# Marcus-Forte/moptimizer_0

Measured on NVIDIA B200. Metric: point2point_linearized_residuals_per_sec, higher is better.
Workload: dtype f32

## Files before the change

moptimizer_0_b200/csrc/mopt_capi.cu:

```cuda
#include <dlfcn.h>

#include <cmath>
#include <atomic>
#include <chrono>
#include <cstdlib>
#include <cstring>
#include <mutex>

#include "mopt_internal.h"

using namespace mopt;

namespace {
thread_local std::string g_last_error;
}
namespace mopt {
void set_last_error(const std::string& msg) { g_last_error = msg; }
int store_upload_async(mopt_store* st, int group, const void* host, int host_dtype, int64_t host_stride, int64_t first,
                       int64_t count);
}

namespace {
struct NcclApi {
  typedef struct ncclComm* comm_t;
// ... 170 lines not shown

void fill_cost(const mopt_problem* p, CostDev* c) {
  std::memset(c, 0, sizeof(*c));
  c->model = p->model; c->variant = p->variant; c->P = p->num_parameters; c->O = p->num_outputs;
  c->jacobian = p->jacobian; c->loss = p->loss; c->has_cov = p->has_covariance ? 1 : 0;
  c->compute_dtype = p->compute_dtype; c->loss_param = p->loss_param;
  c->manifold = p->manifold;
  c->rot_offset = (p->model == MOPT_MODEL_POINT2POINT || p->model == MOPT_MODEL_PINHOLE ||
                   p->model == MOPT_MODEL_PINHOLE_DISTORT) ? 3 : -1;
  if (p->model >= MOPT_MODEL_USER_BASE) c->rot_offset = user_model_rot_offset(p->model);
  c->so3_guard = ((p->flags & MOPT_FLAG_REFERENCE_FLOAT_GUARD) && p->compute_dtype == MOPT_F32) ? kSo3GuardF32 : kSo3GuardF64;
  const int O = p->num_outputs;
  for (int i = 0; i < O * O; ++i) c->cov[i] = p->has_covariance ? p->covariance[i] : ((i % (O + 1) == 0) ? 1.0 : 0.0);
  std::memcpy(c->consts, p->consts, sizeof(c->consts));
}

int stage_cost(mopt_ctx* ctx, int i, const mopt_problem* p) {
  CostDev c;
  fill_cost(p, &c);
  if (ctx->cached_valid[i] && std::memcmp(&c, &ctx->cached_cost[i], sizeof(c)) == 0) return MOPT_OK;
  MOPT_CUDA_TRY(cudaStreamSynchronize(ctx->stream));
  ctx->h_slot->cost = c;
  MOPT_CUDA_TRY(cudaMemcpyAsync(&ctx->d_slots[i].cost, &ctx->h_slot->cost, sizeof(CostDev), cudaMemcpyHostToDevice, ctx->stream));
  MOPT_CUDA_TRY(cudaStreamSynchronize(ctx->stream));
  ctx->cached_cost[i] = c;
  ctx->cached_valid[i] = true;
  return MOPT_OK;
}

PassArgs make_args(mopt_ctx* ctx, const mopt_store* st, int slot, int accumulate, int mode_override) {
  PassArgs a;
  std::memset(&a, 0, sizeof(a));
  for (int s = 0; s < kMaxStreams; ++s) a.streams.p[s] = st->streams[s];
  a.n = st->n;
  a.pb = &ctx->d_slots[slot].pb;
  a.cost = &ctx->d_slots[slot].cost;
  a.partials = ctx->d_partials;
  a.ticket = ctx->d_ticket;
  a.out = ctx->d_trial;
  a.accumulate = accumulate;
  a.mode_ptr = &ctx->d_lm->pass_mode;
  a.mode_override = mode_override;
  a.masked = st->may_have_invalid ? 1 : 0;
  return a;
}

bool can_fuse_setup(const mopt_ctx* ctx, const mopt_problem* p, const mopt_store* st) {
  static const int env = [] {
    const char* e = getenv("MOPT_FUSED_SETUP");
    return (e && e[0]) ? (e[0] == '0' ? 0 : 1) : -1;
  }();
  if (env == 0) return false;
  if (p->model == MOPT_MODEL_EXP_CURVE && p->jacobian != MOPT_JAC_ANALYTICAL && st->dtype == MOPT_F32 &&
      p->compute_dtype == MOPT_F32 && !(p->flags & MOPT_FLAG_GENERIC_KERNEL) && !p->has_covariance &&
      !st->may_have_invalid && ctx->threads != 1024)
    return true;
  return p->model == MOPT_MODEL_POINT2POINT && p->jacobian == MOPT_JAC_ANALYTICAL &&
         p->manifold == MOPT_MANIFOLD_ADDITIVE;
}

int launch_pass(mopt_ctx* ctx, const mopt_store* st, const mopt_problem* p, int slot, int accumulate, int mode_override,
                bool push, const XArg* fused_x = nullptr) {
  PassArgs a = make_args(ctx, st, slot, accumulate, mode_override);
  if (fused_x) {
    a.fused_setup = 1;
    a.x = *fused_x;
  }
  if (push && ctx->world > 1 && ctx->peers_open && ctx->exchange_enabled) {
    for (int r = 0; r < ctx->world; ++r) a.peer.base[r] = ctx->peer_base[r];
    a.peer.world = ctx->world;
    a.peer.rank = ctx->rank;
    a.peer.push = 1;
    a.peer.fused = ctx->fused_consumer ? 1 : 0;
    a.peer.err = ctx->d_xerr;
    a.peer.err_dev = ctx->d_xerr_dev;
    a.peer.seq = ++ctx->xseq;
  }
  PassLaunch L{ctx->stream, ctx->num_sms, ctx->ctas_per_sm, ctx->threads};
  L.affine_fd = (p->compute_dtype == MOPT_F32) ? !(p->flags & MOPT_FLAG_GENERIC_KERNEL)
                                               : ((p->flags & MOPT_FLAG_STABLE_FD) && !(p->flags & MOPT_FLAG_GENERIC_KERNEL));
  L.identity_cov = !p->has_covariance;
  if (p->model >= MOPT_MODEL_USER_BASE)
    return launch_user(L, ctx->device, p->model, p->jacobian != MOPT_JAC_ANALYTICAL, st->dtype, p->compute_dtype, a);
  if (p->model == MOPT_MODEL_POINT2POINT && p->jacobian == MOPT_JAC_ANALYTICAL)
    return launch_p2p_moment(L, st->dtype, p->compute_dtype, p->loss,
                             p->variant == MOPT_P2P_EXACT || p->variant == MOPT_P2P_LEFT, a);
  if (p->model == MOPT_MODEL_POINT2POINT && !(p->flags & MOPT_FLAG_GENERIC_KERNEL) &&
      !(st->dtype == MOPT_F64 && p->compute_dtype == MOPT_F32))
    return launch_p2p_moment(L, st->dtype, p->compute_dtype, p->loss, false, a);
  if (p->model == MOPT_MODEL_PINHOLE_DISTORT) return launch_wide(L, p->model, st->dtype, p->compute_dtype, a);
  return launch_dense(L, p->model, p->jacobian != MOPT_JAC_ANALYTICAL, st->dtype, p->compute_dtype, a);
}

int allreduce_trial(mopt_ctx* ctx, int P, int mode_override) {
  if (ctx->world <= 1 || !ctx->exchange_enabled) return MOPT_OK;
  if (ctx->peers_open) {
    if (ctx->fused_consumer) return MOPT_OK;
    peer_reduce_kernel<<<1, 64, 0, ctx->stream>>>(ctx->d_xbuf, ctx->world, ctx->xseq, ctx->d_trial, packed_size(P),
                                                  &ctx->d_lm->pass_mode, mode_override, ctx->d_xerr, ctx->d_xerr_dev);
    MOPT_CUDA_TRY(cudaGetLastError());
    return MOPT_OK;
  }
  if (!ctx->nccl_comm) {
    set_last_error("sharded context has neither a NCCL communicator nor an open peer exchange");
    return MOPT_ERR_COMM;
  }
  MOPT_NCCL_TRY(nccl().AllReduce(ctx->d_trial, ctx->d_trial, size_t(packed_size(P)), kNcclFloat64, kNcclSum,
                                 static_cast<NcclApi::comm_t>(ctx->nccl_comm), ctx->stream));
  return MOPT_OK;
}

void unpack_result(const PassResult& r, int P, double* H, double* b, double* sum) {
  if (H)
    for (int i = 0; i < P; ++i)
// ... 10 lines not shown
int check_exchange_alive(const mopt_ctx* ctx) {
  if (ctx->h_xerr && *reinterpret_cast<volatile int*>(ctx->h_xerr)) {
    set_last_error("an earlier peer exchange on this context timed out (a rank died); destroy the context");
    return MOPT_ERR_COMM;
  }
  return MOPT_OK;
}

int enqueue_pass(mopt_ctx* ctx, mopt_store* st, const mopt_problem* p, const double* x, int mode) {
  MOPT_TRY(check_exchange_alive(ctx));
  MOPT_CUDA_TRY(cudaSetDevice(ctx->device));
  MOPT_TRY(stage_cost(ctx, 0, p));
  const int P = p->num_parameters;
  XArg xa;
  std::memset(&xa, 0, sizeof(xa));
  if (P > 0) {
    MOPT_REQUIRE(x != nullptr, "null parameter vector");
    for (int i = 0; i < P; ++i) xa.v[i] = x[i];
  }
  if (can_fuse_setup(ctx, p, st)) {
    MOPT_TRY(launch_pass(ctx, st, p, 0, 0, mode, true, &xa));
  } else {
    setup_kernel<<<1, 32, 0, ctx->stream>>>(&ctx->d_slots[0], xa);
    MOPT_CUDA_TRY(cudaGetLastError());
    if (user_model_has_setup(p->model))
      MOPT_TRY(launch_user_setup(ctx->stream, ctx->device, p->model, &ctx->d_slots[0], nullptr, xa.v, P));
    MOPT_TRY(launch_pass(ctx, st, p, 0, 0, mode, true));
  }
  MOPT_TRY(allreduce_trial(ctx, P, mode));
  return MOPT_OK;
}

}

namespace mopt {
int setup_slot(mopt_ctx* ctx, int slot, const mopt_problem* problem, const double* x) {
  MOPT_TRY(stage_cost(ctx, slot, problem));
  XArg xa;
  std::memset(&xa, 0, sizeof(xa));
  for (int i = 0; i < problem->num_parameters; ++i) xa.v[i] = x[i];
  setup_kernel<<<1, 32, 0, ctx->stream>>>(&ctx->d_slots[slot], xa);
  MOPT_CUDA_TRY(cudaGetLastError());
  if (user_model_has_setup(problem->model))
    MOPT_TRY(launch_user_setup(ctx->stream, ctx->device, problem->model, &ctx->d_slots[slot], nullptr, xa.v,
                               problem->num_parameters));
  return MOPT_OK;
}
}

namespace {

int fetch_result(mopt_ctx* ctx, int P, double* H, double* b, double* sum) {
  MOPT_CUDA_TRY(cudaMemcpyAsync(ctx->h_result, ctx->d_trial, sizeof(double) * packed_size(P), cudaMemcpyDeviceToHost, ctx->stream));
  MOPT_CUDA_TRY(cudaStreamSynchronize(ctx->stream));
  if (ctx->h_xerr && *reinterpret_cast<volatile int*>(ctx->h_xerr)) {
    set_last_error("peer exchange timed out waiting for another rank");
    return MOPT_ERR_COMM;
  }
  unpack_result(*ctx->h_result, P, H, b, sum);
  return MOPT_OK;
}

int finish_lm(mopt_ctx* ctx, int P, double* x, mopt_lm_report* report, bool on_host = false) {
  LmState* hs = ctx->h_lm;
  constexpr int kFirstTrials = 48;
  const size_t first = offsetof(LmState, trials) + sizeof(mopt_lm_trial) * kFirstTrials;
  if (!on_host) {
    MOPT_CUDA_TRY(cudaMemcpyAsync(hs, ctx->d_lm, first, cudaMemcpyDeviceToHost, ctx->stream));
    MOPT_CUDA_TRY(cudaStreamSynchronize(ctx->stream));
  }
  if (!on_host && hs->num_trials > kFirstTrials) {
    const int more = (hs->num_trials < MOPT_MAX_TRACE ? hs->num_trials : MOPT_MAX_TRACE) - kFirstTrials;
    MOPT_CUDA_TRY(cudaMemcpyAsync(reinterpret_cast<char*>(hs) + first, reinterpret_cast<const char*>(ctx->d_lm) + first,
                                  sizeof(mopt_lm_trial) * size_t(more), cudaMemcpyDeviceToHost, ctx->stream));
    MOPT_CUDA_TRY(cudaStreamSynchronize(ctx->stream));
  }
// ... 286 lines not shown

int mopt_lm_minimize(mopt_ctx* ctx, int n_costs, mopt_store* const* stores, const mopt_problem* problems,
                     const mopt_lm_options* options, double* x, mopt_lm_report* report) try {
  MOPT_REQUIRE(ctx && stores && problems && x && report, "null argument");
  if (n_costs <= 0) {
    set_last_error("No cost function added!");
    return MOPT_ERR_INVALID_ARGUMENT;
  }
  MOPT_REQUIRE(n_costs <= MOPT_MAX_COSTS, "too many cost terms");
  mopt_lm_options opt;
  if (options) opt = *options; else mopt_lm_default_options(&opt);
  MOPT_REQUIRE(opt.max_iterations >= 0, "Optimization::max_iterations cannot be less than 0.");
  MOPT_REQUIRE(opt.lm_max_iterations >= 0, "lm_max_iterations cannot be negative");
  const int P = problems[0].num_parameters;
  MOPT_REQUIRE(P > 0 && P <= kMaxP, "bad num_parameters");
  for (int c = 0; c < n_costs; ++c) {
    MOPT_REQUIRE(stores[c] && stores[c]->ctx == ctx, "store does not belong to this context");
    MOPT_TRY(validate_problem(stores[c], &problems[c], true));
    MOPT_REQUIRE(problems[c].num_parameters == P, "all cost terms must share the parameter vector");
    MOPT_REQUIRE(problems[c].manifold == problems[0].manifold, "all cost terms must use the same manifold");
  }
  MOPT_TRY(check_exchange_alive(ctx));
  MOPT_CUDA_TRY(cudaSetDevice(ctx->device));
  std::memset(report, 0, offsetof(mopt_lm_report, trials));
  if (opt.max_iterations == 0) {
    report->status = MOPT_MAXIMUM_ITERATIONS_REACHED;
    return MOPT_OK;
  }
  for (int c = 0; c < n_costs; ++c) MOPT_TRY(stage_cost(ctx, c, &problems[c]));

  LmInit in;
  std::memset(&in, 0, sizeof(in));
  in.P = P; in.n_costs = n_costs; in.max_it = opt.max_iterations; in.lm_max_it = opt.lm_max_iterations;
  in.speculative = opt.speculative ? 1 : 0; in.scalar_f32 = (opt.scalar_dtype == MOPT_F32) ? 1 : 0;
  bool has_update = false;
  for (int c = 0; c < n_costs; ++c) has_update = has_update || (stores[c]->index != nullptr);
  if (has_update) in.speculative = 0;
  in.lambda_factor = opt.lambda_factor;
  in.flags = opt.flags;
  for (int i = 0; i < P; ++i) in.x0[i] = x[i];
  bool init_launched = false;
  auto launch_init = [&]() -> int {
    if (init_launched) return MOPT_OK;
    lm_init_kernel<<<1, 32, 0, ctx->stream>>>(ctx->d_lm, ctx->d_slots, in);
    MOPT_CUDA_TRY(cudaGetLastError());
    init_launched = true;
// ... 214 lines not shown
```

moptimizer_0_b200/csrc/mopt_icp.cu:

```cuda
#include <cmath>
#include <cstring>
#include <vector>

#include "mopt_internal.h"

using namespace mopt;

struct mopt_nn_index {
  mopt_ctx* ctx = nullptr;
  int dtype = MOPT_F64;
  int64_t m = 0;
  double max_dist = 0.0, cell = 0.0;
  double origin[3] = {0, 0, 0};
  int dims[3] = {1, 1, 1};
  int64_t ncells = 1;
  void* d_pts = nullptr;
  int* d_orig = nullptr;
  unsigned int* d_start = nullptr;
  long long* d_matched = nullptr;
};

namespace {

struct GridDesc {
// ... 154 lines not shown
    if (best_pos != 0xffffffffu) {
      tx[i] = ST(px[best_pos]);
      ty[i] = ST(py[best_pos]);
      tz[i] = ST(pz[best_pos]);
      ++local;
    } else {
      const ST no_match = ST(__longlong_as_double(0x7ff8000000000000LL));
      tx[i] = no_match;
      ty[i] = no_match;
      tz[i] = no_match;
    }
  }
  for (int off = 16; off >= 1; off >>= 1) local += __shfl_xor_sync(0xffffffffu, local, off);
  if ((threadIdx.x & 31) == 0 && local) atomicAdd(reinterpret_cast<unsigned long long*>(matched), (unsigned long long)local);
}

template <typename T>
int build_index(mopt_nn_index* ix, const void* host, int host_dtype) {
  mopt_ctx* ctx = ix->ctx;
  const int64_t m = ix->m;
  const size_t esz = sizeof(T);
  T* d_aos = nullptr;
  MOPT_CUDA_TRY(cudaMalloc(&d_aos, esz * 3 * size_t(m > 0 ? m : 1)));
  if ((host_dtype == MOPT_F32) == (sizeof(T) == 4)) {
    MOPT_CUDA_TRY(cudaMemcpyAsync(d_aos, host, esz * 3 * size_t(m), cudaMemcpyHostToDevice, ctx->stream));
  } else {
    std::vector<T> tmp(size_t(m) * 3);
    if (host_dtype == MOPT_F32) { const float* h = static_cast<const float*>(host); for (size_t i = 0; i < tmp.size(); ++i) tmp[i] = T(h[i]); }
    else { const double* h = static_cast<const double*>(host); for (size_t i = 0; i < tmp.size(); ++i) tmp[i] = T(h[i]); }
    MOPT_CUDA_TRY(cudaMemcpyAsync(d_aos, tmp.data(), esz * 3 * size_t(m), cudaMemcpyHostToDevice, ctx->stream));
    MOPT_CUDA_TRY(cudaStreamSynchronize(ctx->stream));
  }
  const int bb_blocks = 296;
  double* d_part = nullptr;
  MOPT_CUDA_TRY(cudaMalloc(&d_part, sizeof(double) * 6 * bb_blocks));
  bbox_kernel<T><<<bb_blocks, 256, 0, ctx->stream>>>(d_aos, m, d_part);
  MOPT_CUDA_TRY(cudaGetLastError());
  std::vector<double> part(6 * bb_blocks);
  MOPT_CUDA_TRY(cudaMemcpyAsync(part.data(), d_part, sizeof(double) * part.size(), cudaMemcpyDeviceToHost, ctx->stream));
  MOPT_CUDA_TRY(cudaStreamSynchronize(ctx->stream));
  cudaFree(d_part);
  double lo[3] = {1e300, 1e300, 1e300}, hi[3] = {-1e300, -1e300, -1e300};
  for (int b = 0; b < bb_blocks; ++b)
    for (int k = 0; k < 3; ++k) {
      lo[k] = std::fmin(lo[k], part[b * 6 + k]);
      hi[k] = std::fmax(hi[k], part[b * 6 + 3 + k]);
// ... 50 lines not shown

template <typename ST, typename T>
void launch_reassoc(mopt_store* st, mopt_nn_index* ix, const ParamBlock* pb, const LmState* gate) {
  GridDesc g;
  for (int k = 0; k < 3; ++k) { g.origin[k] = ix->origin[k]; g.dims[k] = ix->dims[k]; }
  g.inv_cell = 1.0 / ix->cell;
  const T* pts = static_cast<const T*>(ix->d_pts);
  int blocks = int(std::min<int64_t>((st->n + 255) / 256, 148 * 32));
  if (blocks < 1) blocks = 1;
  reassociate_kernel<ST, T><<<blocks, 256, 0, st->ctx->stream>>>(
      static_cast<const ST*>(st->streams[0]), static_cast<const ST*>(st->streams[1]), static_cast<const ST*>(st->streams[2]),
      static_cast<ST*>(st->streams[3]), static_cast<ST*>(st->streams[4]), static_cast<ST*>(st->streams[5]), st->n, pb, g,
      ix->max_dist, pts, pts + ix->m, pts + 2 * ix->m, ix->d_orig, ix->d_start, ix->d_matched, gate);
}

}

namespace mopt {

int enqueue_reassociate(mopt_store* st, const ParamBlock* pb, const LmState* gate) {
  mopt_nn_index* ix = st->index;
  if (!ix) return MOPT_OK;
  MOPT_CUDA_TRY(cudaMemsetAsync(ix->d_matched, 0, sizeof(long long), st->ctx->stream));
  if (st->dtype == MOPT_F32 && ix->dtype == MOPT_F32) launch_reassoc<float, float>(st, ix, pb, gate);
  else if (st->dtype == MOPT_F32 && ix->dtype == MOPT_F64) launch_reassoc<float, double>(st, ix, pb, gate);
  else if (st->dtype == MOPT_F64 && ix->dtype == MOPT_F32) launch_reassoc<double, float>(st, ix, pb, gate);
  else launch_reassoc<double, double>(st, ix, pb, gate);
  MOPT_CUDA_TRY(cudaGetLastError());
  st->may_have_invalid = true;
  return MOPT_OK;
}

}

extern "C" {

int mopt_nn_index_create(mopt_ctx* ctx, const void* host_xyz, int host_dtype, int index_dtype, int64_t m,
                         double max_distance, mopt_nn_index** out) try {
  MOPT_REQUIRE(ctx && out && (host_xyz || m == 0), "null argument");
  MOPT_REQUIRE(m >= 0 && m < (int64_t(1) << 31), "target cloud size must be below 2^31");
  MOPT_REQUIRE(max_distance > 0.0 && std::isfinite(max_distance), "max_distance must be positive");
  MOPT_REQUIRE((host_dtype == MOPT_F32 || host_dtype == MOPT_F64) && (index_dtype == MOPT_F32 || index_dtype == MOPT_F64),
               "bad dtype");
  MOPT_CUDA_TRY(cudaSetDevice(ctx->device));
  mopt_nn_index* ix = new mopt_nn_index();
  ix->ctx = ctx;
// ... 53 lines not shown
```

moptimizer_0_b200/csrc/mopt_internal.h:

```cpp
#pragma once

#include <cuda_runtime.h>

#include "mopt_common.cuh"
#include "mopt_lm.cuh"
#include "mopt_lm_mono.cuh"
#include "mopt_models.cuh"
#include "mopt_pass.cuh"

struct mopt_ctx {
  int device = 0;
  int num_sms = 148;
  cudaStream_t stream = nullptr;
  cudaStream_t copy_stream = nullptr;
  double* d_partials = nullptr;
  unsigned int* d_ticket = nullptr;
  mopt::PassResult* d_trial = nullptr;
  mopt::CostSlot* d_slots = nullptr;
  mopt::LmState* d_lm = nullptr;
  mopt::PassResult* h_result = nullptr;
  mopt::LmState* h_lm = nullptr;
  mopt::LmState* d_lm_host = nullptr;
  mopt::CostSlot* h_slot = nullptr;
  int* h_flags = nullptr;
// ... 1 lines not shown
  int flags_capacity = 0;
  mopt::CostDev cached_cost[MOPT_MAX_COSTS];
  bool cached_valid[MOPT_MAX_COSTS] = {false};
  void* d_stage[2] = {nullptr, nullptr};
  size_t stage_bytes = 0;
  cudaEvent_t ev_copy[2] = {nullptr, nullptr};
  cudaEvent_t ev_free[2] = {nullptr, nullptr};
  cudaEvent_t ev_batch[2] = {nullptr, nullptr};
  int ctas_per_sm = 0;
  int threads = 0;
  void* nccl_comm = nullptr;
  int rank = 0, world = 1;
  mopt::XSlot* d_xbuf = nullptr;
  mopt::XSlot* peer_base[mopt::kMaxWorld] = {nullptr};
  bool peers_open = false;
  bool exchange_enabled = true;
  bool fused_consumer = true;
  unsigned long long xseq = 0;
  int* h_xerr = nullptr;
  int* d_xerr = nullptr;
  unsigned long long* d_gen = nullptr;
  unsigned long long mono_gen = 0;
  int* d_xerr_dev = nullptr;
};

struct mopt_store {
  mopt_ctx* ctx = nullptr;
  int model = 0;
  int dtype = 0;
  int64_t n = 0;
  int nstreams = 0;
  void* streams[mopt::kMaxStreams] = {nullptr};
  struct mopt_nn_index* index = nullptr;
  bool may_have_invalid = false;
};

namespace mopt {

struct PassLaunch {
  cudaStream_t stream;
  int num_sms;
  int ctas_per_sm;
  int threads;
  bool affine_fd = true;
  bool identity_cov = false;
};

int launch_p2p_moment(const PassLaunch& L, int store_dtype, int compute_dtype, int loss, bool qrot, const PassArgs& a);
int launch_p2p_moment_gen2(const PassLaunch& L, int loss, bool qrot, const PassArgs& a);
int launch_p2p_lm_mono(const PassLaunch& L, int store_dtype, int compute_dtype, int loss, bool qrot, const PassArgs& a,
                       const MonoArgs& m);
int launch_dense(const PassLaunch& L, int model, bool numeric, int store_dtype, int compute_dtype, const PassArgs& a);

int setup_slot(mopt_ctx* ctx, int slot, const mopt_problem* problem, const double* x);
int enqueue_reassociate(mopt_store* st, const ParamBlock* pb, const LmState* gate);

int launch_wide(const PassLaunch& L, int model, int store_dtype, int compute_dtype, const PassArgs& a);

int launch_user(const PassLaunch& L, int device, int model, bool numeric, int store_dtype, int compute_dtype,
                const PassArgs& a);
int launch_user_setup(cudaStream_t stream, int device, int model, CostSlot* slot, const double* x_dev,
                      const double* x_host, int P);
int user_model_rot_offset(int model);
bool user_model_has_setup(int model);

int pick_grid(const void* kernel, int threads, const PassLaunch& L, int64_t work_items);

}
```

moptimizer_0_b200/csrc/mopt_pass_p2p2.cu:

```cuda
#include "mopt_internal.h"
#include "mopt_pass_p2p2.cuh"

namespace mopt {
namespace {

struct ShapeGen2 {
  static constexpr int THREADS = 384, STAGES = 2, U = 2, FLUSH = 16;
};

template <int LOSS, bool QROT, bool MASKED, bool FUSED, class S>
int launch_gen2_one(const PassLaunch& L, const PassArgs& a0) {
  auto kern = p2p_moment2_kernel<LOSS, QROT, MASKED, FUSED, S::THREADS, 1, S::STAGES, S::U, S::FLUSH, 0>;
  constexpr size_t smem = p2p2_ring_bytes(S::THREADS, S::STAGES, S::U);
  static bool configured[64] = {false};
  int dev = 0;
  MOPT_CUDA_TRY(cudaGetDevice(&dev));
  if (dev < 0 || dev >= 64 || !configured[dev]) {
    MOPT_CUDA_TRY(cudaFuncSetAttribute(kern, cudaFuncAttributeMaxDynamicSharedMemorySize, int(smem)));
    if (dev >= 0 && dev < 64) configured[dev] = true;
  }
  PassArgs a = a0;
  for (int k = 0; k < 6; ++k)
    if (reinterpret_cast<uintptr_t>(a.streams.p[k]) & 15u) a.no_ring = 1;
  const int64_t groups = a.n / 4;
  int64_t grid = int64_t(L.ctas_per_sm > 0 ? L.ctas_per_sm : 1) * L.num_sms;
  if (grid > L.num_sms) grid = L.num_sms;
  const int64_t need = (groups + S::THREADS - 1) / S::THREADS;
  if (need < grid) grid = need;
  if (grid < 1) grid = 1;
  kern<<<int(grid), S::THREADS, smem, L.stream>>>(a);
  MOPT_CUDA_TRY(cudaGetLastError());
  return MOPT_OK;
}

template <int LOSS, bool QROT, class S>
int launch_gen2_flags(const PassLaunch& L, const PassArgs& a) {
  if (a.masked)
    return a.fused_setup ? launch_gen2_one<LOSS, QROT, true, true, S>(L, a) : launch_gen2_one<LOSS, QROT, true, false, S>(L, a);
  return a.fused_setup ? launch_gen2_one<LOSS, QROT, false, true, S>(L, a) : launch_gen2_one<LOSS, QROT, false, false, S>(L, a);
}

template <class S>
int launch_gen2(const PassLaunch& L, int loss, bool qrot, const PassArgs& a) {
  switch (loss) {
    case MOPT_LOSS_NONE:
      return qrot ? launch_gen2_flags<MOPT_LOSS_NONE, true, S>(L, a) : launch_gen2_flags<MOPT_LOSS_NONE, false, S>(L, a);
    case MOPT_LOSS_GEMAN_MCCLURE:
      return qrot ? launch_gen2_flags<MOPT_LOSS_GEMAN_MCCLURE, true, S>(L, a)
                  : launch_gen2_flags<MOPT_LOSS_GEMAN_MCCLURE, false, S>(L, a);
    case MOPT_LOSS_HUBER:
      return qrot ? launch_gen2_flags<MOPT_LOSS_HUBER, true, S>(L, a) : launch_gen2_flags<MOPT_LOSS_HUBER, false, S>(L, a);
    default:
      set_last_error("unknown loss kind");
      return MOPT_ERR_INVALID_ARGUMENT;
// ... 11 lines not shown
```

moptimizer_0_b200/csrc/mopt_pass_p2p2.cuh:

```cuda
#pragma once

#include "mopt_pass.cuh"

namespace mopt {
#ifdef __CUDACC__

__device__ __forceinline__ float2 bc2(float a) { return make_float2(a, a); }
__device__ __forceinline__ float2 neg2(float2 a) { return make_float2(-a.x, -a.y); }
__device__ __forceinline__ float2 fma2(float2 a, float2 b, float2 c) { return __ffma2_rn(a, b, c); }
__device__ __forceinline__ float2 add2(float2 a, float2 b) { return __fadd2_rn(a, b); }
__device__ __forceinline__ float2 sub2(float2 a, float2 b) { return __fadd2_rn(a, neg2(b)); }
__device__ __forceinline__ float2 mul2(float2 a, float2 b) { return __fmul2_rn(a, b); }

__device__ __forceinline__ unsigned smem_u32(const void* p) { return static_cast<unsigned>(__cvta_generic_to_shared(p)); }
__device__ __forceinline__ void mbar_init(uint64_t* bar, unsigned count) {
  asm volatile("mbarrier.init.shared::cta.b64 [%0], %1;" ::"r"(smem_u32(bar)), "r"(count) : "memory");
}
__device__ __forceinline__ void mbar_expect_tx(uint64_t* bar, unsigned bytes) {
  asm volatile("mbarrier.arrive.expect_tx.shared::cta.b64 _, [%0], %1;" ::"r"(smem_u32(bar)), "r"(bytes) : "memory");
}
__device__ __forceinline__ void mbar_arrive(uint64_t* bar) {
  asm volatile("mbarrier.arrive.shared::cta.b64 _, [%0];" ::"r"(smem_u32(bar)) : "memory");
}
__device__ __forceinline__ void mbar_wait(uint64_t* bar, unsigned parity) {
  asm volatile(
      "{\n"
      ".reg .pred p;\n"
      "MOPT_WAIT:\n"
      "mbarrier.try_wait.parity.shared::cta.b64 p, [%0], %1;\n"
      "@p bra MOPT_DONE;\n"
      "bra MOPT_WAIT;\n"
      "MOPT_DONE:\n"
      "}\n" ::"r"(smem_u32(bar)),
      "r"(parity)
      : "memory");
}
__device__ __forceinline__ void bulk_g2s(void* dst, const void* src, unsigned bytes, uint64_t* bar) {
  asm volatile("cp.async.bulk.shared::cluster.global.mbarrier::complete_tx::bytes [%0], [%1], %2, [%3];" ::"r"(smem_u32(dst)),
               "l"(src), "r"(bytes), "r"(smem_u32(bar))
               : "memory");
}

template <int LOSS>
__device__ __forceinline__ float loss_weight_fast(float k, float e2) {
  if constexpr (LOSS == MOPT_LOSS_HUBER) {
    float rs;
    asm("rsqrt.approx.ftz.f32 %0, %1;" : "=f"(rs) : "f"(fmaxf(e2, 1.17549435e-38f)));
    return (e2 <= k * k) ? 1.0f : k * rs;
  } else {
    return loss_weight<float>(LOSS, k, e2);
  }
}

template <int LOSS, bool QROT, bool MASKED>
__device__ __forceinline__ void p2p_moments_x2(const float (&R)[9], const float (&t)[3], float lossp, float2 px, float2 py,
                                               float2 pz, float2 yx, float2 yy, float2 yz, float2 (&acc)[kP2PRaw]) {
  bool skip0 = false, skip1 = false;
  if constexpr (MASKED) {
    skip0 = yx.x != yx.x; skip1 = yx.y != yx.y;
    if (skip0) { px.x = py.x = pz.x = 0.f; yx.x = t[0]; yy.x = t[1]; yz.x = t[2]; }
    if (skip1) { px.y = py.y = pz.y = 0.f; yx.y = t[0]; yy.y = t[1]; yz.y = t[2]; }
  }
  const float2 q0 = fma2(px, bc2(R[0]), fma2(py, bc2(R[1]), mul2(pz, bc2(R[2]))));
  const float2 q1 = fma2(px, bc2(R[3]), fma2(py, bc2(R[4]), mul2(pz, bc2(R[5]))));
// ... 21 lines not shown
  acc[19] = fma2(w2, r0, acc[19]); acc[20] = fma2(w2, r1, acc[20]); acc[21] = fma2(w2, r2, acc[21]);
  acc[22] = add2(acc[22], e2);
}

template <bool MASKED>
__device__ __forceinline__ void p2p_cost_x2(const float (&R)[9], const float (&t)[3], float2 px, float2 py, float2 pz,
                                            float2 yx, float2 yy, float2 yz, float2 (&acc)[kP2PRaw]) {
  const float2 r0 = sub2(add2(fma2(px, bc2(R[0]), fma2(py, bc2(R[1]), mul2(pz, bc2(R[2])))), bc2(t[0])), yx);
  const float2 r1 = sub2(add2(fma2(px, bc2(R[3]), fma2(py, bc2(R[4]), mul2(pz, bc2(R[5])))), bc2(t[1])), yy);
  const float2 r2 = sub2(add2(fma2(px, bc2(R[6]), fma2(py, bc2(R[7]), mul2(pz, bc2(R[8])))), bc2(t[2])), yz);
  float2 e2 = fma2(r0, r0, fma2(r1, r1, mul2(r2, r2)));
  if constexpr (MASKED) {
    if (yx.x != yx.x) e2.x = 0.f;
    if (yx.y != yx.y) e2.y = 0.f;
  }
  acc[22] = add2(acc[22], e2);
}

constexpr size_t p2p2_ring_bytes(int threads, int stages, int u) { return size_t(stages) * 6 * size_t(u) * threads * 16; }

template <int LOSS, bool QROT, bool MASKED, bool FUSED, int THREADS, int MINB, int STAGES, int U, int FLUSH_ROUNDS,
          int PF = 0>
__global__ void __launch_bounds__(THREADS, MINB) p2p_moment2_kernel(const PassArgs a) {
  const int mode = a.mode_override >= 0 ? a.mode_override : *a.mode_ptr;
  if (mode == PASS_SKIP) return;
  if (peer_failed(a)) return;
  constexpr int NW = THREADS / 32;
  constexpr int CHUNK = THREADS * U;

  __shared__ double s_warp[NW * 32];
  __shared__ double s_tot[32];
  __shared__ double s_set0[FUSED ? 12 : 1];
  __shared__ __align__(8) uint64_t s_full[STAGES > 0 ? STAGES : 1];
  __shared__ __align__(8) uint64_t s_empty[STAGES > 0 ? STAGES : 1];
  extern __shared__ __align__(128) unsigned char p2p2_ring[];
  float4* ring = reinterpret_cast<float4*>(p2p2_ring);

  const int lane = threadIdx.x & 31;
  const double* set0 = FUSED ? s_set0 : a.pb->sets[0];
  if constexpr (FUSED) {
    if (threadIdx.x == 0) {
      double xl[6];
#pragma unroll
      for (int i = 0; i < 6; ++i) xl[i] = a.x.v[i];
      p2p_fused_set0(a.cost, xl, s_set0);
    }
// ... 135 lines not shown
    for (int64_t g = full_rounds * stride + int64_t(blockIdx.x) * THREADS + threadIdx.x; g < ngroups;
         g += int64_t(gridDim.x) * THREADS) {
      direct_group(g);
      if (++since_flush >= FLUSH_ROUNDS) {
        flush();
        since_flush = 0;
      }
    }
    if (blockIdx.x == 0 && threadIdx.x == 0) {
      for (int64_t i = ngroups * 4; i < a.n; ++i) {
        float2 one[kP2PRaw];
#pragma unroll
        for (int k = 0; k < kP2PRaw; ++k) one[k] = make_float2(0.f, 0.f);
        const float2 px = make_float2(sp[0][i], 0.f), py = make_float2(sp[1][i], 0.f), pz = make_float2(sp[2][i], 0.f);
        const float2 yx = make_float2(sp[3][i], t[0]), yy = make_float2(sp[4][i], t[1]), yz = make_float2(sp[5][i], t[2]);
        if (mode == PASS_COST) p2p_cost_x2<MASKED>(R, t, px, py, pz, yx, yy, yz, one);
        else p2p_moments_x2<LOSS, QROT, MASKED>(R, t, lossp, px, py, pz, yx, yy, yz, one);
#pragma unroll
        for (int k = 0; k < kP2PRaw; ++k) acc[k].x += one[k].x;
      }
    }
  }
  flush();
  p2p_finish<FUSED, THREADS>(a, mode, dacc, s_tot, s_warp);
}

#endif
}
```

moptimizer_0_b200/csrc/mopt_peaks.cu:

```cuda
#include <algorithm>
#include <chrono>
#include <cstring>
#include <vector>

#include "mopt_internal.h"

namespace {

using namespace mopt;

template <int ILP>
__global__ void __launch_bounds__(512) fma_peak_kernel(const float* bc, float* out, int iters) {
  const float b = bc[0], c = bc[1];
  float a[ILP];
#pragma unroll
  for (int k = 0; k < ILP; ++k) a[k] = float(threadIdx.x + k) * 1e-3f;
  for (int i = 0; i < iters; ++i) {
#pragma unroll
    for (int k = 0; k < ILP; ++k) a[k] = fmaf(a[k], b, c);
  }
  float s = 0.f;
#pragma unroll
  for (int k = 0; k < ILP; ++k) s += a[k];
  if (s == 123.456f) out[0] = s;
// ... 43 lines not shown
  for (int r = 0; r < reps; ++r) {
    MOPT_CUDA_TRY(cudaEventRecord(e0, stream));
    launch();
    MOPT_CUDA_TRY(cudaEventRecord(e1, stream));
    MOPT_CUDA_TRY(cudaEventSynchronize(e1));
    float ms = 0.f;
    MOPT_CUDA_TRY(cudaEventElapsedTime(&ms, e0, e1));
    best = std::min(best, ms);
  }
  cudaEventDestroy(e0);
  cudaEventDestroy(e1);
  MOPT_CUDA_TRY(cudaGetLastError());
  *best_ms = best;
  return MOPT_OK;
}

}

extern "C" int mopt_measure_peaks(mopt_ctx* ctx, mopt_peaks* out) try {
  MOPT_REQUIRE(ctx && out, "null argument");
  MOPT_CUDA_TRY(cudaSetDevice(ctx->device));
  std::memset(out, 0, sizeof(*out));
  cudaStream_t s = ctx->stream;
  float *d_bc = nullptr, *d_out = nullptr;
  MOPT_CUDA_TRY(cudaMalloc(&d_bc, 2 * sizeof(float)));
  MOPT_CUDA_TRY(cudaMalloc(&d_out, sizeof(float)));
  const float bc[2] = {0.999f, 1e-3f};
  MOPT_CUDA_TRY(cudaMemcpy(d_bc, bc, sizeof(bc), cudaMemcpyHostToDevice));
  constexpr int ILP = 8, THREADS = 512;
  const int grid = ctx->num_sms * 4;
  const int iters = 20000;
  const double thread_ops = double(grid) * THREADS * double(iters) * ILP;
  float ms = 0.f;
  MOPT_TRY(time_best(s, [&] { fma_peak_kernel<ILP><<<grid, THREADS, 0, s>>>(d_bc, d_out, iters); }, 5, &ms));
  out->fp32_fma_tflops = 2.0 * thread_ops / (ms * 1e-3) / 1e12;
  MOPT_TRY(time_best(s, [&] { fma2_peak_kernel<ILP><<<grid, THREADS, 0, s>>>(d_bc, d_out, iters); }, 5, &ms));
  out->fp32_fma2_tflops = 4.0 * thread_ops / (ms * 1e-3) / 1e12;
  out->issue_gwarp_inst_per_s = out->fp32_fma_tflops * 1e12 / 64.0 / 1e9;
  {
    const int64_t bytes = int64_t(2) << 30;
    float4* buf = nullptr;
    MOPT_CUDA_TRY(cudaMalloc(&buf, size_t(bytes)));
    MOPT_CUDA_TRY(cudaMemsetAsync(buf, 0, size_t(bytes), s));
    const int64_t n4 = bytes / 16;
    MOPT_TRY(time_best(s, [&] { read_peak_kernel<<<ctx->num_sms * 8, 256, 0, s>>>(buf, n4, d_out); }, 10, &ms));
    out->hbm_read_gbs = double(bytes) / (ms * 1e-3) / 1e9;
    cudaFree(buf);
  }
  cudaFree(d_bc);
  cudaFree(d_out);
  return MOPT_OK;
}
MOPT_ABI_CATCH

extern "C" int mopt_measure_h2d(mopt_ctx* ctx, uint64_t bytes, double seconds, double* gbs) try {
  MOPT_REQUIRE(ctx && gbs && bytes >= (1u << 20), "bad argument");
  MOPT_CUDA_TRY(cudaSetDevice(ctx->device));
  const size_t chunk = size_t(64) << 20;
  void *h = nullptr, *d = nullptr;
  MOPT_CUDA_TRY(cudaHostAlloc(&h, bytes, cudaHostAllocDefault));
  std::memset(h, 1, bytes);
  if (cudaMalloc(&d, bytes) != cudaSuccess) {
    cudaFreeHost(h);
    (void)cudaGetLastError();
    mopt::set_last_error("mopt_measure_h2d: out of device memory");
    return MOPT_ERR_OUT_OF_MEMORY;
  }
  cudaStream_t s = ctx->stream;
  auto sweep = [&] {
    for (size_t o = 0; o < bytes; o += chunk)
      cudaMemcpyAsync(static_cast<char*>(d) + o, static_cast<char*>(h) + o, std::min(chunk, size_t(bytes) - o),
                      cudaMemcpyHostToDevice, s);
  };
  sweep();
  MOPT_CUDA_TRY(cudaStreamSynchronize(s));
  const auto t0 = std::chrono::steady_clock::now();
  double elapsed = 0.0;
  uint64_t moved = 0;
  do {
    sweep();
    MOPT_CUDA_TRY(cudaStreamSynchronize(s));
    moved += bytes;
    elapsed = std::chrono::duration<double>(std::chrono::steady_clock::now() - t0).count();
  } while (elapsed < seconds);
  *gbs = double(moved) / elapsed / 1e9;
  cudaFree(d);
  cudaFreeHost(h);
  return MOPT_OK;
}
MOPT_ABI_CATCH
```

moptimizer_0_b200/csrc/mopt_store.cu:

```cuda
#include <cstring>

#include "mopt_internal.h"

using namespace mopt;

namespace {

template <typename HT, typename ST>
__global__ void deinterleave_kernel(const HT* __restrict__ aos, int64_t stride, int ncomp, ST* __restrict__ s0,
                                    ST* __restrict__ s1, ST* __restrict__ s2, int64_t first, int64_t count) {
  for (int64_t i = int64_t(blockIdx.x) * blockDim.x + threadIdx.x; i < count; i += int64_t(gridDim.x) * blockDim.x) {
    const HT* e = aos + i * stride;
    s0[first + i] = ST(e[0]);
    if (ncomp > 1) s1[first + i] = ST(e[1]);
    if (ncomp > 2) s2[first + i] = ST(e[2]);
  }
}

template <typename HT, typename ST>
__global__ void interleave_kernel(HT* __restrict__ aos, int ncomp, const ST* __restrict__ s0, const ST* __restrict__ s1,
                                  const ST* __restrict__ s2, int64_t first, int64_t count) {
  for (int64_t i = int64_t(blockIdx.x) * blockDim.x + threadIdx.x; i < count; i += int64_t(gridDim.x) * blockDim.x) {
    HT* e = aos + i * ncomp;
    e[0] = HT(s0[first + i]);
// ... 141 lines not shown

namespace mopt {

int store_upload_async(mopt_store* st, int group, const void* host, int host_dtype, int64_t host_stride, int64_t first,
                       int64_t count) {
  mopt_ctx* ctx = st->ctx;
  const ModelShape sh = model_shape(st->model);
  MOPT_REQUIRE(group == 0 || group == 1, "group must be 0 (A) or 1 (B)");
  const int ncomp = group == 0 ? sh.ncomp_a : sh.ncomp_b;
  MOPT_REQUIRE(ncomp > 0, "this model has no such data group");
  MOPT_REQUIRE(first >= 0 && count >= 0 && first + count <= st->n, "upload range outside the store");
  MOPT_REQUIRE(host_dtype == MOPT_F32 || host_dtype == MOPT_F64, "bad host dtype");
  if (count == 0) return MOPT_OK;
  MOPT_REQUIRE(host != nullptr, "null host pointer");
  if (host_stride == 0) host_stride = ncomp;
  MOPT_REQUIRE(host_stride >= ncomp, "host stride smaller than the component count");
  void* const* streams = st->streams + (group == 0 ? 0 : sh.NA);
  const size_t hsz = dtype_size(host_dtype);
  const size_t chunk_bytes_target = size_t(64) << 20;
  int64_t chunk_elems = int64_t(chunk_bytes_target / (hsz * size_t(host_stride)));
  if (chunk_elems < 1) chunk_elems = 1;
  if (chunk_elems > count) chunk_elems = count;
  MOPT_TRY(ensure_stage(ctx, size_t(chunk_elems) * size_t(host_stride) * hsz));
  int buf = 0;
  for (int64_t off = 0; off < count; off += chunk_elems, buf ^= 1) {
    const int64_t m = (count - off < chunk_elems) ? (count - off) : chunk_elems;
    const size_t bytes = (size_t(m - 1) * size_t(host_stride) + size_t(ncomp)) * hsz;
    MOPT_CUDA_TRY(cudaStreamWaitEvent(ctx->copy_stream, ctx->ev_free[buf], 0));
    MOPT_CUDA_TRY(cudaMemcpyAsync(ctx->d_stage[buf], static_cast<const char*>(host) + size_t(off) * size_t(host_stride) * hsz,
                                  bytes, cudaMemcpyHostToDevice, ctx->copy_stream));
    MOPT_CUDA_TRY(cudaEventRecord(ctx->ev_copy[buf], ctx->copy_stream));
    MOPT_CUDA_TRY(cudaStreamWaitEvent(ctx->stream, ctx->ev_copy[buf], 0));
    if (host_dtype == MOPT_F32 && st->dtype == MOPT_F32)
      launch_deinterleave<float, float>(ctx->stream, ctx->d_stage[buf], host_stride, ncomp, streams, first + off, m);
    else if (host_dtype == MOPT_F64 && st->dtype == MOPT_F32)
      launch_deinterleave<double, float>(ctx->stream, ctx->d_stage[buf], host_stride, ncomp, streams, first + off, m);
    else if (host_dtype == MOPT_F32 && st->dtype == MOPT_F64)
      launch_deinterleave<float, double>(ctx->stream, ctx->d_stage[buf], host_stride, ncomp, streams, first + off, m);
    else
      launch_deinterleave<double, double>(ctx->stream, ctx->d_stage[buf], host_stride, ncomp, streams, first + off, m);
    MOPT_CUDA_TRY(cudaGetLastError());
    MOPT_CUDA_TRY(cudaEventRecord(ctx->ev_free[buf], ctx->stream));
  }
  return MOPT_OK;
}

// ... 52 lines not shown
  MOPT_CUDA_TRY(cudaSetDevice(st->ctx->device));
  MOPT_TRY(store_upload_async(st, group, host, host_dtype, host_stride, first, count));
  MOPT_CUDA_TRY(cudaStreamSynchronize(st->ctx->stream));
  return MOPT_OK;
}
MOPT_ABI_CATCH

int mopt_store_download(mopt_store* st, int group, void* host, int host_dtype, int64_t first, int64_t count) try {
  MOPT_REQUIRE(st && host, "null store/host");
  mopt_ctx* ctx = st->ctx;
  MOPT_CUDA_TRY(cudaSetDevice(ctx->device));
  const ModelShape sh = model_shape(st->model);
  MOPT_REQUIRE(group == 0 || group == 1, "group must be 0 (A) or 1 (B)");
  const int ncomp = group == 0 ? sh.ncomp_a : sh.ncomp_b;
  MOPT_REQUIRE(ncomp > 0, "this model has no such data group");
  MOPT_REQUIRE(first >= 0 && count >= 0 && first + count <= st->n, "download range outside the store");
  MOPT_REQUIRE(host_dtype == MOPT_F32 || host_dtype == MOPT_F64, "bad host dtype");
  void* const* streams = st->streams + (group == 0 ? 0 : sh.NA);
  const size_t hsz = dtype_size(host_dtype);
  const int64_t chunk_elems_max = int64_t((size_t(64) << 20) / (hsz * ncomp));
  const int64_t chunk = count < chunk_elems_max ? count : chunk_elems_max;
  if (count == 0) return MOPT_OK;
  MOPT_TRY(ensure_stage(ctx, size_t(chunk) * ncomp * hsz));
  for (int64_t off = 0; off < count; off += chunk) {
    const int64_t m = (count - off < chunk) ? (count - off) : chunk;
    if (host_dtype == MOPT_F32 && st->dtype == MOPT_F32)
      launch_interleave<float, float>(ctx->stream, ctx->d_stage[0], ncomp, streams, first + off, m);
    else if (host_dtype == MOPT_F64 && st->dtype == MOPT_F32)
      launch_interleave<double, float>(ctx->stream, ctx->d_stage[0], ncomp, streams, first + off, m);
    else if (host_dtype == MOPT_F32 && st->dtype == MOPT_F64)
      launch_interleave<float, double>(ctx->stream, ctx->d_stage[0], ncomp, streams, first + off, m);
    else
      launch_interleave<double, double>(ctx->stream, ctx->d_stage[0], ncomp, streams, first + off, m);
    MOPT_CUDA_TRY(cudaGetLastError());
    MOPT_CUDA_TRY(cudaMemcpyAsync(static_cast<char*>(host) + size_t(off) * ncomp * hsz, ctx->d_stage[0],
                                  size_t(m) * ncomp * hsz, cudaMemcpyDeviceToHost, ctx->stream));
    MOPT_CUDA_TRY(cudaStreamSynchronize(ctx->stream));
  }
  return MOPT_OK;
}
MOPT_ABI_CATCH

int mopt_store_generate(mopt_store* st, const mopt_synth* desc) try {
  MOPT_REQUIRE(st && desc, "null store/desc");
  mopt_ctx* ctx = st->ctx;
  MOPT_CUDA_TRY(cudaSetDevice(ctx->device));
  SynthDev d;
  std::memset(&d, 0, sizeof(d));
  d.seed = desc->seed;
  d.first_index = desc->first_index;
  d.n_total = desc->n_total > 0 ? desc->n_total : st->n;
  for (int k = 0; k < 3; ++k) {
    d.lo[k] = float(desc->lo[k]);
    d.hi[k] = float(desc->hi[k]);
  }
  d.sigma = float(desc->noise_sigma);
  d.outlier_fraction = float(desc->outlier_fraction);
  d.outlier_range = float(desc->outlier_range);
  const int threads = 256;
  int64_t blocks = (st->n + threads - 1) / threads;
  if (blocks > 148 * 16) blocks = 148 * 16;
  if (blocks < 1) blocks = 1;
  const bool f32 = st->dtype == MOPT_F32;
  switch (st->model) {
    case MOPT_MODEL_POINT2POINT:
    case MOPT_MODEL_POINT_DIST: {
      double R[9];
      rodrigues_host(desc->gt + 3, R);
      for (int i = 0; i < 9; ++i) d.gt[i] = float(R[i]);
      for (int i = 0; i < 3; ++i) d.gt[9 + i] = float(desc->gt[i]);
      if (f32)
        generate_p2p_kernel<float><<<int(blocks), threads, 0, ctx->stream>>>(
            d, st->n, (float*)st->streams[0], (float*)st->streams[1], (float*)st->streams[2], (float*)st->streams[3],
            (float*)st->streams[4], (float*)st->streams[5]);
      else
        generate_p2p_kernel<double><<<int(blocks), threads, 0, ctx->stream>>>(
            d, st->n, (double*)st->streams[0], (double*)st->streams[1], (double*)st->streams[2], (double*)st->streams[3],
            (double*)st->streams[4], (double*)st->streams[5]);
      break;
    }
    case MOPT_MODEL_EXP_CURVE: {
      d.gt[0] = float(desc->gt[0]);
      d.gt[1] = float(desc->gt[1]);
      if (f32)
        generate_curve_kernel<float><<<int(blocks), threads, 0, ctx->stream>>>(d, st->n, (float*)st->streams[0],
                                                                               (float*)st->streams[1]);
// ... 43 lines not shown
```

Before: 287.7.

## Use programmatic dependent launch between back-to-back point2point moment passes

Result: no change. 290.3, median of 6 (+0.9%).

```diff
diff --git a/moptimizer_0_b200/csrc/mopt_capi.cu b/moptimizer_0_b200/csrc/mopt_capi.cu
--- a/moptimizer_0_b200/csrc/mopt_capi.cu
+++ b/moptimizer_0_b200/csrc/mopt_capi.cu
@@ -216,6 +216,7 @@
   MOPT_CUDA_TRY(cudaStreamSynchronize(ctx->stream));
   ctx->h_slot->cost = c;
   MOPT_CUDA_TRY(cudaMemcpyAsync(&ctx->d_slots[i].cost, &ctx->h_slot->cost, sizeof(CostDev), cudaMemcpyHostToDevice, ctx->stream));
+  note_stream_work(ctx, false);
   MOPT_CUDA_TRY(cudaStreamSynchronize(ctx->stream));
   ctx->cached_cost[i] = c;
   ctx->cached_valid[i] = true;
@@ -253,6 +254,19 @@
          p->manifold == MOPT_MANIFOLD_ADDITIVE;
 }
 
+int dispatch_pass(const PassLaunch& L, int device, const mopt_store* st, const mopt_problem* p, const PassArgs& a) {
+  if (p->model >= MOPT_MODEL_USER_BASE)
+    return launch_user(L, device, p->model, p->jacobian != MOPT_JAC_ANALYTICAL, st->dtype, p->compute_dtype, a);
+  if (p->model == MOPT_MODEL_POINT2POINT && p->jacobian == MOPT_JAC_ANALYTICAL)
+    return launch_p2p_moment(L, st->dtype, p->compute_dtype, p->loss,
+                             p->variant == MOPT_P2P_EXACT || p->variant == MOPT_P2P_LEFT, a);
+  if (p->model == MOPT_MODEL_POINT2POINT && !(p->flags & MOPT_FLAG_GENERIC_KERNEL) &&
+      !(st->dtype == MOPT_F64 && p->compute_dtype == MOPT_F32))
+    return launch_p2p_moment(L, st->dtype, p->compute_dtype, p->loss, false, a);
+  if (p->model == MOPT_MODEL_PINHOLE_DISTORT) return launch_wide(L, p->model, st->dtype, p->compute_dtype, a);
+  return launch_dense(L, p->model, p->jacobian != MOPT_JAC_ANALYTICAL, st->dtype, p->compute_dtype, a);
+}
+
 int launch_pass(mopt_ctx* ctx, const mopt_store* st, const mopt_problem* p, int slot, int accumulate, int mode_override,
                 bool push, const XArg* fused_x = nullptr) {
   PassArgs a = make_args(ctx, st, slot, accumulate, mode_override);
@@ -274,16 +288,12 @@
   L.affine_fd = (p->compute_dtype == MOPT_F32) ? !(p->flags & MOPT_FLAG_GENERIC_KERNEL)
                                                : ((p->flags & MOPT_FLAG_STABLE_FD) && !(p->flags & MOPT_FLAG_GENERIC_KERNEL));
   L.identity_cov = !p->has_covariance;
-  if (p->model >= MOPT_MODEL_USER_BASE)
-    return launch_user(L, ctx->device, p->model, p->jacobian != MOPT_JAC_ANALYTICAL, st->dtype, p->compute_dtype, a);
-  if (p->model == MOPT_MODEL_POINT2POINT && p->jacobian == MOPT_JAC_ANALYTICAL)
-    return launch_p2p_moment(L, st->dtype, p->compute_dtype, p->loss,
-                             p->variant == MOPT_P2P_EXACT || p->variant == MOPT_P2P_LEFT, a);
-  if (p->model == MOPT_MODEL_POINT2POINT && !(p->flags & MOPT_FLAG_GENERIC_KERNEL) &&
-      !(st->dtype == MOPT_F64 && p->compute_dtype == MOPT_F32))
-    return launch_p2p_moment(L, st->dtype, p->compute_dtype, p->loss, false, a);
-  if (p->model == MOPT_MODEL_PINHOLE_DISTORT) return launch_wide(L, p->model, st->dtype, p->compute_dtype, a);
-  return launch_dense(L, p->model, p->jacobian != MOPT_JAC_ANALYTICAL, st->dtype, p->compute_dtype, a);
+  L.after_gen2 = ctx->gen2_tail;
+  bool gen2 = false;
+  L.gen2_launched = &gen2;
+  const int r = dispatch_pass(L, ctx->device, st, p, a);
+  note_stream_work(ctx, r == MOPT_OK && gen2 && ctx->world == 1 && mode_override >= 0);
+  return r;
 }
 
 int allreduce_trial(mopt_ctx* ctx, int P, int mode_override) {
@@ -340,6 +350,7 @@
     MOPT_TRY(launch_pass(ctx, st, p, 0, 0, mode, true, &xa));
   } else {
     setup_kernel<<<1, 32, 0, ctx->stream>>>(&ctx->d_slots[0], xa);
+    note_stream_work(ctx, false);
     MOPT_CUDA_TRY(cudaGetLastError());
     if (user_model_has_setup(p->model))
       MOPT_TRY(launch_user_setup(ctx->stream, ctx->device, p->model, &ctx->d_slots[0], nullptr, xa.v, P));
@@ -358,6 +369,7 @@
   std::memset(&xa, 0, sizeof(xa));
   for (int i = 0; i < problem->num_parameters; ++i) xa.v[i] = x[i];
   setup_kernel<<<1, 32, 0, ctx->stream>>>(&ctx->d_slots[slot], xa);
+  note_stream_work(ctx, false);
   MOPT_CUDA_TRY(cudaGetLastError());
   if (user_model_has_setup(problem->model))
     MOPT_TRY(launch_user_setup(ctx->stream, ctx->device, problem->model, &ctx->d_slots[slot], nullptr, xa.v,
@@ -370,6 +382,7 @@
 
 int fetch_result(mopt_ctx* ctx, int P, double* H, double* b, double* sum) {
   MOPT_CUDA_TRY(cudaMemcpyAsync(ctx->h_result, ctx->d_trial, sizeof(double) * packed_size(P), cudaMemcpyDeviceToHost, ctx->stream));
+  note_stream_work(ctx, false);
   MOPT_CUDA_TRY(cudaStreamSynchronize(ctx->stream));
   if (ctx->h_xerr && *reinterpret_cast<volatile int*>(ctx->h_xerr)) {
     set_last_error("peer exchange timed out waiting for another rank");
@@ -702,6 +715,7 @@
   }
   MOPT_TRY(check_exchange_alive(ctx));
   MOPT_CUDA_TRY(cudaSetDevice(ctx->device));
+  note_stream_work(ctx, false);
   std::memset(report, 0, offsetof(mopt_lm_report, trials));
   if (opt.max_iterations == 0) {
     report->status = MOPT_MAXIMUM_ITERATIONS_REACHED;
diff --git a/moptimizer_0_b200/csrc/mopt_icp.cu b/moptimizer_0_b200/csrc/mopt_icp.cu
--- a/moptimizer_0_b200/csrc/mopt_icp.cu
+++ b/moptimizer_0_b200/csrc/mopt_icp.cu
@@ -200,6 +200,7 @@
   const size_t esz = sizeof(T);
   T* d_aos = nullptr;
   MOPT_CUDA_TRY(cudaMalloc(&d_aos, esz * 3 * size_t(m > 0 ? m : 1)));
+  note_stream_work(ctx, false);
   if ((host_dtype == MOPT_F32) == (sizeof(T) == 4)) {
     MOPT_CUDA_TRY(cudaMemcpyAsync(d_aos, host, esz * 3 * size_t(m), cudaMemcpyHostToDevice, ctx->stream));
   } else {
@@ -296,6 +297,7 @@
   mopt_nn_index* ix = st->index;
   if (!ix) return MOPT_OK;
   MOPT_CUDA_TRY(cudaMemsetAsync(ix->d_matched, 0, sizeof(long long), st->ctx->stream));
+  note_stream_work(st->ctx, false);
   if (st->dtype == MOPT_F32 && ix->dtype == MOPT_F32) launch_reassoc<float, float>(st, ix, pb, gate);
   else if (st->dtype == MOPT_F32 && ix->dtype == MOPT_F64) launch_reassoc<float, double>(st, ix, pb, gate);
   else if (st->dtype == MOPT_F64 && ix->dtype == MOPT_F32) launch_reassoc<double, float>(st, ix, pb, gate);
diff --git a/moptimizer_0_b200/csrc/mopt_internal.h b/moptimizer_0_b200/csrc/mopt_internal.h
--- a/moptimizer_0_b200/csrc/mopt_internal.h
+++ b/moptimizer_0_b200/csrc/mopt_internal.h
@@ -47,6 +47,7 @@
   unsigned long long* d_gen = nullptr;
   unsigned long long mono_gen = 0;
   int* d_xerr_dev = nullptr;
+  bool gen2_tail = false;
 };
 
 struct mopt_store {
@@ -69,6 +70,8 @@
   int threads;
   bool affine_fd = true;
   bool identity_cov = false;
+  bool after_gen2 = false;
+  bool* gen2_launched = nullptr;
 };
 
 int launch_p2p_moment(const PassLaunch& L, int store_dtype, int compute_dtype, int loss, bool qrot, const PassArgs& a);
@@ -91,4 +94,6 @@
 
 int pick_grid(const void* kernel, int threads, const PassLaunch& L, int64_t work_items);
 
+inline void note_stream_work(mopt_ctx* ctx, bool gen2_pass) { ctx->gen2_tail = gen2_pass; }
+
 }
diff --git a/moptimizer_0_b200/csrc/mopt_pass_p2p2.cu b/moptimizer_0_b200/csrc/mopt_pass_p2p2.cu
--- a/moptimizer_0_b200/csrc/mopt_pass_p2p2.cu
+++ b/moptimizer_0_b200/csrc/mopt_pass_p2p2.cu
@@ -28,8 +28,18 @@
   const int64_t need = (groups + S::THREADS - 1) / S::THREADS;
   if (need < grid) grid = need;
   if (grid < 1) grid = 1;
-  kern<<<int(grid), S::THREADS, smem, L.stream>>>(a);
-  MOPT_CUDA_TRY(cudaGetLastError());
+  cudaLaunchAttribute attr;
+  attr.id = cudaLaunchAttributeProgrammaticStreamSerialization;
+  attr.val.programmaticStreamSerializationAllowed = 1;
+  cudaLaunchConfig_t cfg = {};
+  cfg.gridDim = dim3(unsigned(grid));
+  cfg.blockDim = dim3(S::THREADS);
+  cfg.dynamicSmemBytes = smem;
+  cfg.stream = L.stream;
+  cfg.attrs = &attr;
+  cfg.numAttrs = L.after_gen2 ? 1 : 0;
+  MOPT_CUDA_TRY(cudaLaunchKernelEx(&cfg, kern, a));
+  if (L.gen2_launched) *L.gen2_launched = true;
   return MOPT_OK;
 }
 
diff --git a/moptimizer_0_b200/csrc/mopt_pass_p2p2.cuh b/moptimizer_0_b200/csrc/mopt_pass_p2p2.cuh
--- a/moptimizer_0_b200/csrc/mopt_pass_p2p2.cuh
+++ b/moptimizer_0_b200/csrc/mopt_pass_p2p2.cuh
@@ -40,6 +40,9 @@
                "l"(src), "r"(bytes), "r"(smem_u32(bar))
                : "memory");
 }
+
+__device__ __forceinline__ void pdl_launch_dependents() { asm volatile("griddepcontrol.launch_dependents;" ::: "memory"); }
+__device__ __forceinline__ void pdl_wait() { asm volatile("griddepcontrol.wait;" ::: "memory"); }
 
 template <int LOSS>
 __device__ __forceinline__ float loss_weight_fast(float k, float e2) {
@@ -107,6 +110,7 @@
 template <int LOSS, bool QROT, bool MASKED, bool FUSED, int THREADS, int MINB, int STAGES, int U, int FLUSH_ROUNDS,
           int PF = 0>
 __global__ void __launch_bounds__(THREADS, MINB) p2p_moment2_kernel(const PassArgs a) {
+  pdl_launch_dependents();
   const int mode = a.mode_override >= 0 ? a.mode_override : *a.mode_ptr;
   if (mode == PASS_SKIP) return;
   if (peer_failed(a)) return;
@@ -288,6 +292,7 @@
     }
   }
   flush();
+  pdl_wait();
   p2p_finish<FUSED, THREADS>(a, mode, dacc, s_tot, s_warp);
 }
 
diff --git a/moptimizer_0_b200/csrc/mopt_peaks.cu b/moptimizer_0_b200/csrc/mopt_peaks.cu
--- a/moptimizer_0_b200/csrc/mopt_peaks.cu
+++ b/moptimizer_0_b200/csrc/mopt_peaks.cu
@@ -89,6 +89,7 @@
   MOPT_CUDA_TRY(cudaSetDevice(ctx->device));
   std::memset(out, 0, sizeof(*out));
   cudaStream_t s = ctx->stream;
+  mopt::note_stream_work(ctx, false);
   float *d_bc = nullptr, *d_out = nullptr;
   MOPT_CUDA_TRY(cudaMalloc(&d_bc, 2 * sizeof(float)));
   MOPT_CUDA_TRY(cudaMalloc(&d_out, sizeof(float)));
@@ -134,6 +135,7 @@
     return MOPT_ERR_OUT_OF_MEMORY;
   }
   cudaStream_t s = ctx->stream;
+  mopt::note_stream_work(ctx, false);
   auto sweep = [&] {
     for (size_t o = 0; o < bytes; o += chunk)
       cudaMemcpyAsync(static_cast<char*>(d) + o, static_cast<char*>(h) + o, std::min(chunk, size_t(bytes) - o),
diff --git a/moptimizer_0_b200/csrc/mopt_store.cu b/moptimizer_0_b200/csrc/mopt_store.cu
--- a/moptimizer_0_b200/csrc/mopt_store.cu
+++ b/moptimizer_0_b200/csrc/mopt_store.cu
@@ -187,6 +187,7 @@
   if (chunk_elems < 1) chunk_elems = 1;
   if (chunk_elems > count) chunk_elems = count;
   MOPT_TRY(ensure_stage(ctx, size_t(chunk_elems) * size_t(host_stride) * hsz));
+  note_stream_work(ctx, false);
   int buf = 0;
   for (int64_t off = 0; off < count; off += chunk_elems, buf ^= 1) {
     const int64_t m = (count - off < chunk_elems) ? (count - off) : chunk_elems;
@@ -285,6 +286,7 @@
   const int64_t chunk = count < chunk_elems_max ? count : chunk_elems_max;
   if (count == 0) return MOPT_OK;
   MOPT_TRY(ensure_stage(ctx, size_t(chunk) * ncomp * hsz));
+  note_stream_work(ctx, false);
   for (int64_t off = 0; off < count; off += chunk) {
     const int64_t m = (count - off < chunk) ? (count - off) : chunk;
     if (host_dtype == MOPT_F32 && st->dtype == MOPT_F32)
@@ -325,6 +327,7 @@
   if (blocks > 148 * 16) blocks = 148 * 16;
   if (blocks < 1) blocks = 1;
   const bool f32 = st->dtype == MOPT_F32;
+  note_stream_work(ctx, false);
   switch (st->model) {
     case MOPT_MODEL_POINT2POINT:
     case MOPT_MODEL_POINT_DIST: {
```
